# SonyCSLParis/interactive-spectrogram-inpainting

Hardware: AMD Instinct MI355X
Metric: spectrograms/sec VQ-VAE fwd+quantize @B64 (higher is better)
Workload: dtype f32 (products split into two f16 pieces, three terms); 1 GPU; VQVAE.forward (encode + quantize x2 + decode), eval, default ctor (128 hidden, 2 res blocks, D=64, K=512, factors 4/2); batch_per_gpu=64, input=[2,128,512] fp32 randn, weights=random init, codebooks calibrated on encoder outputs, parallelism=replicas x1 (no data-path collective)

## Files before the change

interactive-spectrogram-inpainting_amd/csrc/conv_first_f32.hip:

```cpp
#include <cstdlib>

#include "device_prims.h"
#include "isi_common.h"
#include "isi_internal.h"
#include "knobs.h"
#include "prof.h"
#include "split_f16.h"

namespace isi {

namespace {

constexpr unsigned OOB = 0xFFFFFFF0u;
constexpr int TILES_PER_WAVE = 8;
constexpr int LDT = 68;

struct FirstArgs {
  const float *in, *w, *bias;
  float *out;
  unsigned in_bytes;
  int s0n, s0c, s0h, s0w;
  int H, W, OH, OW, M;
  int relu, out_pair;
  float *out2;
  const float *gate;
  int32_t *zero;
  int zero_words;
};


template <int COUT>
__device__ __forceinline__ void store_tile(const FirstArgs &p, const float *tb, const int m0, const int lane) {
  if (p.out_pair) {
    constexpr int GP = COUT / 8;
    typedef unsigned u32x2v __attribute__((ext_vector_type(2)));
#pragma unroll
    for (int it = 0; it < 32 * GP / 64; ++it) {
      const int idx = it * 64 + lane;
      const int px = idx / GP, g = idx - px * GP;
      uint4 hi, lo;
      f16s::pair8_encode(*reinterpret_cast<const float4 *>(tb + px * LDT + g * 8),
                         *reinterpret_cast<const float4 *>(tb + px * LDT + g * 8 + 4), hi, lo);
      if (!p.out2 && 32 * GP % 64 == 0) {
        const u32x2v sx = __builtin_amdgcn_permlane32_swap(hi.x, lo.x, false, false);
        const u32x2v sy = __builtin_amdgcn_permlane32_swap(hi.y, lo.y, false, false);
        const u32x2v sz = __builtin_amdgcn_permlane32_swap(hi.z, lo.z, false, false);
        const u32x2v sw = __builtin_amdgcn_permlane32_swap(hi.w, lo.w, false, false);
        const uint4 first = make_uint4(sx.x, sy.x, sz.x, sw.x), second = make_uint4(sx.y, sy.y, sz.y, sw.y);
        const int up = lane >> 5;
        const int idx_a = it * 64 + (lane & 31), idx_b = idx_a + 32;
        const int pa = idx_a / GP, ga = idx_a - pa * GP, pb = idx_b / GP, gb = idx_b - pb * GP;
        if (m0 + pa < p.M) reinterpret_cast<uint4 *>(p.out + (size_t)(m0 + pa) * COUT + ga * 8)[up] = first;
        if (m0 + pb < p.M) reinterpret_cast<uint4 *>(p.out + (size_t)(m0 + pb) * COUT + gb * 8)[up] = second;
        continue;
      }
      if (m0 + px < p.M) {
        uint4 *o = reinterpret_cast<uint4 *>(p.out + (size_t)(m0 + px) * COUT + g * 8);
        o[0] = hi;
        o[1] = lo;
        if (p.out2) {
          float4 *o2 = reinterpret_cast<float4 *>(p.out2 + (size_t)(m0 + px) * COUT + g * 8);
          o2[0] = *reinterpret_cast<const float4 *>(tb + px * LDT + g * 8);
          o2[1] = *reinterpret_cast<const float4 *>(tb + px * LDT + g * 8 + 4);
        }
      }
    }
    return;
  }
  constexpr int QP = COUT / 4;
#pragma unroll
  for (int it = 0; it < 32 * QP / 64; ++it) {
    const int idx = it * 64 + lane;
    const int px = idx / QP, q = idx - px * QP;
    if (m0 + px < p.M) {
      float4 v = *reinterpret_cast<const float4 *>(tb + px * LDT + q * 4);
      if (p.gate) {
        const float4 g = *reinterpret_cast<const float4 *>(p.gate + (size_t)(m0 + px) * COUT + q * 4);
        v.x = g.x > 0.f ? v.x : 0.f; v.y = g.y > 0.f ? v.y : 0.f; v.z = g.z > 0.f ? v.z : 0.f; v.w = g.w > 0.f ? v.w : 0.f;
      }
      *reinterpret_cast<float4 *>(p.out + (size_t)(m0 + px) * COUT + q * 4) = v;
    }
  }
}

template <int NT>
__global__ __launch_bounds__(256) void conv_first_kernel(const FirstArgs p) {
  constexpr int COUT = NT * 32;
  __shared__ __attribute__((aligned(16))) float tbuf[4][32 * LDT];
  const int tid = threadIdx.x, lane = tid & 63, wave = tid >> 6;
  const int col = lane & 31, half = lane >> 5;
  float *tb = tbuf[wave];
  if (p.zero && blockIdx.x == 0)
    for (int i = tid; i < p.zero_words; i += 256) p.zero[i] = 0;

  float4 bw[4][NT];
#pragma unroll
  for (int s = 0; s < 4; ++s)
#pragma unroll
    for (int j = 0; j < NT; ++j)
      bw[s][j] = *reinterpret_cast<const float4 *>(p.w + (size_t)(32 * j + col) * 32 + 8 * s + 4 * half);
  float bias[NT];
#pragma unroll
  for (int j = 0; j < NT; ++j) bias[j] = p.bias ? p.bias[32 * j + col] : 0.f;

  const __amdgpu_buffer_rsrc_t rsi = __builtin_amdgcn_make_buffer_rsrc(const_cast<float *>(p.in), 0, p.in_bytes, 0x00020000);
  const int ohw = p.OH * p.OW;

  for (int t = 0; t < TILES_PER_WAVE; ++t) {
    const int tile = (t * (int)gridDim.x + (int)blockIdx.x) * 4 + wave;
    const int m0 = tile * 32;
    const int m = m0 + col;
    float a[4][4];
    {
      const bool ok = m < p.M;
      const int b = ok ? m / ohw : 0;
      const int rem = m - b * ohw;
      const int oy = rem / p.OW, ox = rem - oy * p.OW;
      const int iy0 = 2 * oy - 1, ix0 = 2 * ox - 1 + 2 * half;
      const int base = b * p.s0n;
#pragma unroll
      for (int s = 0; s < 4; ++s) {
        const int iy = iy0 + s;
        const bool yok = ok && (unsigned)iy < (unsigned)p.H;
#pragma unroll
        for (int e = 0; e < 4; ++e) {
          const int ix = ix0 + (e >> 1);
          const bool in_range = yok && (unsigned)ix < (unsigned)p.W;
          const unsigned off = in_range ? (unsigned)(base + (e & 1) * p.s0c + iy * p.s0h + ix * p.s0w) * 4u : OOB;
          a[s][e] = __builtin_bit_cast(float, __builtin_amdgcn_raw_buffer_load_b32(rsi, off, 0, 0));
        }
      }
    }
    f32x16 acc[NT];
#pragma unroll
    for (int j = 0; j < NT; ++j)
#pragma unroll
      for (int r = 0; r < 16; ++r) acc[j][r] = 0.f;
#pragma unroll
    for (int s = 0; s < 4; ++s)
#pragma unroll
      for (int e = 0; e < 4; ++e)
#pragma unroll
        for (int j = 0; j < NT; ++j) {
          const float bv = e == 0 ? bw[s][j].x : e == 1 ? bw[s][j].y : e == 2 ? bw[s][j].z : bw[s][j].w;
          acc[j] = __builtin_amdgcn_mfma_f32_32x32x2f32(a[s][e], bv, acc[j], 0, 0, 0);
        }
    __syncthreads();
#pragma unroll
    for (int j = 0; j < NT; ++j)
#pragma unroll
      for (int r = 0; r < 16; ++r) {
        const int row = (r & 3) + 8 * (r >> 2) + 4 * half;
        float v = acc[j][r] + bias[j];
        if (p.relu) v = fmaxf(v, 0.f) + (v - v);
        tb[row * LDT + 32 * j + col] = v;
      }
    __syncthreads();
    store_tile<COUT>(p, tb, m0, lane);
  }
}

typedef short s16x8f __attribute__((ext_vector_type(8)));
template <int NT>
__global__ __launch_bounds__(256) void conv_first_f16x3_kernel(const FirstArgs p) {
  constexpr int COUT = NT * 32;
  __shared__ __attribute__((aligned(16))) float tbuf[4][32 * LDT];
  const int tid = threadIdx.x, lane = tid & 63, wave = tid >> 6;
  const int col = lane & 31, half = lane >> 5;
  float *tb = tbuf[wave];
  if (p.zero && blockIdx.x == 0)
    for (int i = tid; i < p.zero_words; i += 256) p.zero[i] = 0;

  s16x8f bh[2][NT], bl[2][NT];
#pragma unroll
  for (int st = 0; st < 2; ++st)
#pragma unroll
    for (int j = 0; j < NT; ++j) {
      const float *wr = p.w + (size_t)(32 * j + col) * 32 + 16 * st + 8 * half;
      uint2 h0, l0, h1, l1;
      f16s::split4(*reinterpret_cast<const float4 *>(wr), f16s::kScaleB, h0, l0);
      f16s::split4(*reinterpret_cast<const float4 *>(wr + 4), f16s::kScaleB, h1, l1);
      bh[st][j] = __builtin_bit_cast(s16x8f, make_uint4(h0.x, h0.y, h1.x, h1.y));
      bl[st][j] = __builtin_bit_cast(s16x8f, make_uint4(l0.x, l0.y, l1.x, l1.y));
    }
  float bias[NT];
#pragma unroll
  for (int j = 0; j < NT; ++j) bias[j] = p.bias ? p.bias[32 * j + col] : 0.f;

  const __amdgpu_buffer_rsrc_t rsi = __builtin_amdgcn_make_buffer_rsrc(const_cast<float *>(p.in), 0, p.in_bytes, 0x00020000);
  const int ohw = p.OH * p.OW;

  for (int t = 0; t < TILES_PER_WAVE; ++t) {
    const int tile = (t * (int)gridDim.x + (int)blockIdx.x) * 4 + wave;
    const int m0 = tile * 32;
    const int m = m0 + col;
    float a[2][8];
    {
      const bool ok = m < p.M;
      const int b = ok ? m / ohw : 0;
      const int rem = m - b * ohw;
      const int oy = rem / p.OW, ox = rem - oy * p.OW;
      const int iy0 = 2 * oy - 1 + half, ix0 = 2 * ox - 1;
      const int base = b * p.s0n;
#pragma unroll
      for (int st = 0; st < 2; ++st) {
        const int iy = iy0 + 2 * st;
        const bool yok = ok && (unsigned)iy < (unsigned)p.H;
#pragma unroll
        for (int i = 0; i < 8; ++i) {
          const int ix = ix0 + (i >> 1);
          const bool in_range = yok && (unsigned)ix < (unsigned)p.W;
          const unsigned off = in_range ? (unsigned)(base + (i & 1) * p.s0c + iy * p.s0h + ix * p.s0w) * 4u : OOB;
          a[st][i] = __builtin_bit_cast(float, __builtin_amdgcn_raw_buffer_load_b32(rsi, off, 0, 0));
        }
      }
    }
    f32x16 acc[NT];
#pragma unroll
    for (int j = 0; j < NT; ++j)
#pragma unroll
      for (int r = 0; r < 16; ++r) acc[j][r] = 0.f;
#pragma unroll
    for (int st = 0; st < 2; ++st) {
      uint2 h0, l0, h1, l1;
      f16s::split4(make_float4(a[st][0], a[st][1], a[st][2], a[st][3]), f16s::kScaleA, h0, l0);
      f16s::split4(make_float4(a[st][4], a[st][5], a[st][6], a[st][7]), f16s::kScaleA, h1, l1);
      const s16x8f ah = __builtin_bit_cast(s16x8f, make_uint4(h0.x, h0.y, h1.x, h1.y));
      const s16x8f al = __builtin_bit_cast(s16x8f, make_uint4(l0.x, l0.y, l1.x, l1.y));
#pragma unroll
      for (int j = 0; j < NT; ++j) {
        acc[j] = __builtin_amdgcn_mfma_f32_32x32x16_f16(__builtin_bit_cast(f16s::f16x8, al), __builtin_bit_cast(f16s::f16x8, bh[st][j]), acc[j], 0, 0, 0);
        acc[j] = __builtin_amdgcn_mfma_f32_32x32x16_f16(__builtin_bit_cast(f16s::f16x8, ah), __builtin_bit_cast(f16s::f16x8, bl[st][j]), acc[j], 0, 0, 0);
        acc[j] = __builtin_amdgcn_mfma_f32_32x32x16_f16(__builtin_bit_cast(f16s::f16x8, ah), __builtin_bit_cast(f16s::f16x8, bh[st][j]), acc[j], 0, 0, 0);
      }
    }
    __syncthreads();
#pragma unroll
    for (int j = 0; j < NT; ++j)
#pragma unroll
      for (int r = 0; r < 16; ++r) {
        const int row = (r & 3) + 8 * (r >> 2) + 4 * half;
        float v = acc[j][r] * f16s::kUnscale + bias[j];
        if (p.relu) v = fmaxf(v, 0.f) + (v - v);
        tb[row * LDT + 32 * j + col] = v;
      }
    __syncthreads();
    store_tile<COUT>(p, tb, m0, lane);
  }
}

template <int NT, bool F16>
int launch_first(const FirstArgs &a, hipStream_t stream) {
  const int tiles = (a.M + 31) / 32;
  const int per_wg = 4 * TILES_PER_WAVE;
  dim3 grid((tiles + per_wg - 1) / per_wg);
  const double flops = 2.0 * a.M * (NT * 32) * 32;
  const double bytes = 4.0 * ((double)a.M / (a.OH * a.OW) * 2.0 * a.H * a.W + (double)a.M * NT * 32 + NT * 32 * 32);
  prof::Scope scope(prof::K_CONV_GATHER, flops, bytes, stream);
  if (F16) {
    ISI_PROF_LAUNCH(scope, conv_first_f16x3_kernel<NT>, grid, dim3(256), 0, stream, a);
  } else {
    ISI_PROF_LAUNCH(scope, conv_first_kernel<NT>, grid, dim3(256), 0, stream, a);
  }
  return check_launch("conv_first_f32");
}

}

bool conv_first_applicable(const isi_src *s0, const isi_src *s1, const isi_src *res, const isi_dst *dst, int Cout,
                           int KH, int KW, int stride, int pad, int OH, int OW, int nz) {
  const bool off = knobs().no_conv_first != 0;
  if (off || nz != 1 || (s1 && s1->ptr) || (res && res->ptr)) return false;
  if (s0->C != 2 || KH != 4 || KW != 4 || stride != 2 || pad != 1) return false;
  if (Cout != 32 && Cout != 64) return false;
  if (dst->sc != 1 || dst->sw != Cout || dst->sh != (int64_t)OW * Cout || dst->sn != (int64_t)OH * OW * Cout) return false;
  return (reinterpret_cast<uintptr_t>(dst->ptr) & 15) == 0;
}

int conv_first_f32(const isi_src *s0, const float *packed_w, const float *bias, const isi_dst *dst, int B, int H,
                   int W, int Cout, int OH, int OW, int64_t in_extent, int flags, hipStream_t stream, float *twin,
                   const float *gate, int32_t *zero, int zero_words) {
  FirstArgs a;
  if (zero && zero_words <= 0) return invalid("conv_first: bad zeroing request");
  a.zero = zero; a.zero_words = zero ? zero_words : 0;
  if (twin && !(flags & ISI_CONV_OUT_PAIR)) return unsupported("conv_first: an fp32 twin accompanies a pair-format output");
  if (gate && (flags & (ISI_CONV_OUT_PAIR | ISI_CONV_GATE_PAIR))) return unsupported("conv_first: the gated epilogue writes and reads fp32");
  a.out2 = twin; a.gate = gate;
  a.in = s0->ptr; a.w = packed_w; a.bias = bias; a.out = dst->ptr;
  a.in_bytes = (unsigned)(in_extent * 4);
  a.s0n = (int)s0->sn; a.s0c = (int)s0->sc; a.s0h = (int)s0->sh; a.s0w = (int)s0->sw;
  a.H = H; a.W = W; a.OH = OH; a.OW = OW; a.M = B * OH * OW;
  a.relu = flags & ISI_CONV_RELU; a.out_pair = (flags & ISI_CONV_OUT_PAIR) ? 1 : 0;
  if ((flags & ISI_CONV_F16X3) && !(flags & ISI_CONV_BF16X6))
    return Cout == 64 ? launch_first<2, true>(a, stream) : launch_first<1, true>(a, stream);
  return Cout == 64 ? launch_first<2, false>(a, stream) : launch_first<1, false>(a, stream);
}

}
```

Measured before the change: 37650 spectrograms/s.

## Restructure first conv kernel: row-aligned tiles, vector loads with DPP halo, specialized epilogues

Reworks the first 4x4 stride-2 conv kernel. Tiles now map to 32-pixel row segments, walked incrementally without per-pixel divides. For contiguous inputs each lane does a 64-bit load plus one edge load, and neighbours are exchanged with DPP shifts instead of 16 scalar gathers. The epilogue is specialized by template on mode and ReLU. It swaps the MFMA operands so accumulators can be written transposed to LDS with only wave-local fences instead of block barriers. It also uses buffer stores, stages bias in LDS and prefetches the next tile's input in the f16x3 path. These changes cut address arithmetic, load count and synchronization, at the cost of many more kernel instantiations and more complex edge handling.

```diff
diff --git a/interactive-spectrogram-inpainting_amd/csrc/conv_first_f32.hip b/interactive-spectrogram-inpainting_amd/csrc/conv_first_f32.hip
--- a/interactive-spectrogram-inpainting_amd/csrc/conv_first_f32.hip
+++ b/interactive-spectrogram-inpainting_amd/csrc/conv_first_f32.hip
@@ -21,6 +21,8 @@
   unsigned in_bytes;
   int s0n, s0c, s0h, s0w;
   int H, W, OH, OW, M;
+  int tpr, tiles;
+  int contig;
   int relu, out_pair;
   float *out2;
   const float *gate;
@@ -28,70 +30,164 @@
   int zero_words;
 };
 
-
-template <int COUT>
-__device__ __forceinline__ void store_tile(const FirstArgs &p, const float *tb, const int m0, const int lane) {
-  if (p.out_pair) {
+struct TileWalk {
+  int b, oy, tx;
+  int db, doy, dtx;
+  __device__ __forceinline__ TileWalk(const FirstArgs &p, const int first, const int step) {
+    const int row = first / p.tpr;
+    tx = first - row * p.tpr; b = row / p.OH; oy = row - b * p.OH;
+    const int srow = step / p.tpr;
+    dtx = step - srow * p.tpr; db = srow / p.OH; doy = srow - db * p.OH;
+  }
+  __device__ __forceinline__ void advance(const FirstArgs &p) {
+    tx += dtx; oy += doy; b += db;
+    if (tx >= p.tpr) { tx -= p.tpr; ++oy; }
+    if (oy >= p.OH) { oy -= p.OH; ++b; }
+  }
+};
+
+__device__ __forceinline__ float wave_shr1(const float v) {
+  return __builtin_bit_cast(float, __builtin_amdgcn_update_dpp(0, __builtin_bit_cast(int, v), 0x138, 0xf, 0xf, false));
+}
+__device__ __forceinline__ float wave_shl1(const float v) {
+  return __builtin_bit_cast(float, __builtin_amdgcn_update_dpp(0, __builtin_bit_cast(int, v), 0x130, 0xf, 0xf, false));
+}
+
+struct EdgeLane {
+  bool ok; int ex;
+  __device__ __forceinline__ EdgeLane(const FirstArgs &p, const int col, const int ox0) {
+    ex = col == 0 ? 2 * ox0 - 1 : 2 * ox0 + 64;
+    ok = ((col == 0) | (col == 31)) & ((unsigned)ex < (unsigned)p.W);
+  }
+};
+__device__ __forceinline__ void row4_issue(const __amdgpu_buffer_rsrc_t rsi, const int rowoff, const bool yok, const bool pok,
+                                           const int col, const int ox0, const EdgeLane &el, float (&raw)[3]) {
+  typedef float f32x2v __attribute__((ext_vector_type(2)));
+  const unsigned moff = (yok & pok) ? (unsigned)(rowoff + 2 * (ox0 + col)) * 4u : OOB;
+  const unsigned eoff = (yok & el.ok) ? (unsigned)(rowoff + el.ex) * 4u : OOB;
+  const f32x2v v = __builtin_bit_cast(f32x2v, __builtin_amdgcn_raw_buffer_load_b64(rsi, moff, 0, 0));
+  raw[0] = v.x; raw[1] = v.y;
+  raw[2] = __builtin_bit_cast(float, __builtin_amdgcn_raw_buffer_load_b32(rsi, eoff, 0, 0));
+}
+__device__ __forceinline__ void row4_finish(const float (&raw)[3], const int col, float (&r)[4]) {
+  const float left = wave_shr1(raw[1]), right = wave_shl1(raw[0]);
+  r[0] = col == 0 ? raw[2] : left;
+  r[1] = raw[0];
+  r[2] = raw[1];
+  r[3] = col == 31 ? raw[2] : right;
+}
+template <int N>
+__device__ __forceinline__ void row_elems(const __amdgpu_buffer_rsrc_t rsi, const FirstArgs &p, const int rowoff, const bool yok,
+                                          const bool pok, const int ix0, float (&r)[N]) {
+#pragma unroll
+  for (int k = 0; k < N; ++k) {
+    const int ix = ix0 + k;
+    const bool in_range = yok & pok & ((unsigned)ix < (unsigned)p.W);
+    r[k] = __builtin_bit_cast(float, __builtin_amdgcn_raw_buffer_load_b32(rsi, in_range ? (unsigned)(rowoff + ix * p.s0w) * 4u : OOB, 0, 0));
+  }
+}
+
+enum { EPI_F32 = 0, EPI_GATE = 1, EPI_PAIR = 2, EPI_TWIN = 3 };
+__device__ __forceinline__ void wave_lds_fence() {
+  __builtin_amdgcn_fence(__ATOMIC_RELEASE, "wavefront", "local");
+  __builtin_amdgcn_wave_barrier();
+  __builtin_amdgcn_fence(__ATOMIC_ACQUIRE, "wavefront", "local");
+}
+template <int NT, int MODE, bool RELU, bool SCALED, class MM>
+__device__ __forceinline__ void epilogue(const MM &mm, const float *bsh, float *tb, const __amdgpu_buffer_rsrc_t rso,
+                                         const __amdgpu_buffer_rsrc_t rsx, const int lane) {
+  constexpr int COUT = NT * 32;
+  const int col = lane & 31, half = lane >> 5;
+  typedef unsigned u32x2v __attribute__((ext_vector_type(2)));
+#pragma unroll
+  for (int j = 0; j < NT; ++j) {
+    if (j) __builtin_amdgcn_sched_barrier(0);
+    const f32x16 acc = mm(j);
+#pragma unroll
+    for (int q = 0; q < 4; ++q) {
+      const float4 bq = *reinterpret_cast<const float4 *>(bsh + 32 * j + 8 * q + 4 * half);
+      float v[4];
+#pragma unroll
+      for (int e = 0; e < 4; ++e) {
+        float t = SCALED ? acc[4 * q + e] * f16s::kUnscale + elem(bq, e) : acc[4 * q + e] + elem(bq, e);
+        if (RELU) t = fmaxf(t, 0.f) + (t - t);
+        v[e] = t;
+      }
+      *reinterpret_cast<float4 *>(tb + col * LDT + 32 * j + 8 * q + 4 * half) = make_float4(v[0], v[1], v[2], v[3]);
+    }
+  }
+  wave_lds_fence();
+  if constexpr (MODE == EPI_PAIR || MODE == EPI_TWIN) {
     constexpr int GP = COUT / 8;
-    typedef unsigned u32x2v __attribute__((ext_vector_type(2)));
 #pragma unroll
     for (int it = 0; it < 32 * GP / 64; ++it) {
       const int idx = it * 64 + lane;
       const int px = idx / GP, g = idx - px * GP;
+      const float4 a = *reinterpret_cast<const float4 *>(tb + px * LDT + g * 8), b = *reinterpret_cast<const float4 *>(tb + px * LDT + g * 8 + 4);
       uint4 hi, lo;
-      f16s::pair8_encode(*reinterpret_cast<const float4 *>(tb + px * LDT + g * 8),
-                         *reinterpret_cast<const float4 *>(tb + px * LDT + g * 8 + 4), hi, lo);
-      if (!p.out2 && 32 * GP % 64 == 0) {
+      f16s::pair8_encode(a, b, hi, lo);
+      if constexpr (MODE == EPI_PAIR) {
         const u32x2v sx = __builtin_amdgcn_permlane32_swap(hi.x, lo.x, false, false);
         const u32x2v sy = __builtin_amdgcn_permlane32_swap(hi.y, lo.y, false, false);
         const u32x2v sz = __builtin_amdgcn_permlane32_swap(hi.z, lo.z, false, false);
         const u32x2v sw = __builtin_amdgcn_permlane32_swap(hi.w, lo.w, false, false);
-        const uint4 first = make_uint4(sx.x, sy.x, sz.x, sw.x), second = make_uint4(sx.y, sy.y, sz.y, sw.y);
-        const int up = lane >> 5;
-        const int idx_a = it * 64 + (lane & 31), idx_b = idx_a + 32;
-        const int pa = idx_a / GP, ga = idx_a - pa * GP, pb = idx_b / GP, gb = idx_b - pb * GP;
-        if (m0 + pa < p.M) reinterpret_cast<uint4 *>(p.out + (size_t)(m0 + pa) * COUT + ga * 8)[up] = first;
-        if (m0 + pb < p.M) reinterpret_cast<uint4 *>(p.out + (size_t)(m0 + pb) * COUT + gb * 8)[up] = second;
-        continue;
-      }
-      if (m0 + px < p.M) {
-        uint4 *o = reinterpret_cast<uint4 *>(p.out + (size_t)(m0 + px) * COUT + g * 8);
-        o[0] = hi;
-        o[1] = lo;
-        if (p.out2) {
-          float4 *o2 = reinterpret_cast<float4 *>(p.out2 + (size_t)(m0 + px) * COUT + g * 8);
-          o2[0] = *reinterpret_cast<const float4 *>(tb + px * LDT + g * 8);
-          o2[1] = *reinterpret_cast<const float4 *>(tb + px * LDT + g * 8 + 4);
-        }
-      }
-    }
-    return;
-  }
-  constexpr int QP = COUT / 4;
-#pragma unroll
-  for (int it = 0; it < 32 * QP / 64; ++it) {
-    const int idx = it * 64 + lane;
-    const int px = idx / QP, q = idx - px * QP;
-    if (m0 + px < p.M) {
+        const i32x4 first = {(int)sx.x, (int)sy.x, (int)sz.x, (int)sw.x}, second = {(int)sx.y, (int)sy.y, (int)sz.y, (int)sw.y};
+        const int idx_a = it * 64 + col, idx_b = idx_a + 32;
+        __builtin_amdgcn_raw_buffer_store_b128(first, rso, (unsigned)idx_a * 32u + (unsigned)half * 16u, 0, 0);
+        __builtin_amdgcn_raw_buffer_store_b128(second, rso, (unsigned)idx_b * 32u + (unsigned)half * 16u, 0, 0);
+      } else {
+        __builtin_amdgcn_raw_buffer_store_b128(__builtin_bit_cast(i32x4, hi), rso, (unsigned)idx * 32u, 0, 0);
+        __builtin_amdgcn_raw_buffer_store_b128(__builtin_bit_cast(i32x4, lo), rso, (unsigned)idx * 32u + 16u, 0, 0);
+        __builtin_amdgcn_raw_buffer_store_b128(__builtin_bit_cast(i32x4, a), rsx, (unsigned)idx * 32u, 0, 0);
+        __builtin_amdgcn_raw_buffer_store_b128(__builtin_bit_cast(i32x4, b), rsx, (unsigned)idx * 32u + 16u, 0, 0);
+      }
+    }
+  } else {
+    constexpr int QP = COUT / 4;
+#pragma unroll
+    for (int it = 0; it < 32 * QP / 64; ++it) {
+      const int idx = it * 64 + lane;
+      const int px = idx / QP, q = idx - px * QP;
       float4 v = *reinterpret_cast<const float4 *>(tb + px * LDT + q * 4);
-      if (p.gate) {
-        const float4 g = *reinterpret_cast<const float4 *>(p.gate + (size_t)(m0 + px) * COUT + q * 4);
+      if constexpr (MODE == EPI_GATE) {
+        const float4 g = buf_load4(rsx, (unsigned)idx * 16u);
         v.x = g.x > 0.f ? v.x : 0.f; v.y = g.y > 0.f ? v.y : 0.f; v.z = g.z > 0.f ? v.z : 0.f; v.w = g.w > 0.f ? v.w : 0.f;
       }
-      *reinterpret_cast<float4 *>(p.out + (size_t)(m0 + px) * COUT + q * 4) = v;
-    }
-  }
-}
-
-template <int NT>
-__global__ __launch_bounds__(256) void conv_first_kernel(const FirstArgs p) {
+      __builtin_amdgcn_raw_buffer_store_b128(__builtin_bit_cast(i32x4, v), rso, (unsigned)idx * 16u, 0, 0);
+    }
+  }
+  wave_lds_fence();
+}
+
+template <int NT, bool SCALED, int MODE, bool RELU, class MM>
+__device__ __forceinline__ void store_tile(const FirstArgs &p, const MM &mm, const float *bsh, float *tb, const int b,
+                                           const int oy, const int tx, const int lane) {
   constexpr int COUT = NT * 32;
+  const int ox0 = tx * 32;
+  const int npx = min(32, p.OW - ox0);
+  const size_t first = ((size_t)(b * p.OH + oy) * p.OW + ox0) * COUT;
+  const unsigned bytes = (unsigned)npx * COUT * 4u;
+  const float *x = MODE == EPI_TWIN ? p.out2 : MODE == EPI_GATE ? p.gate : nullptr;
+  const __amdgpu_buffer_rsrc_t rso = __builtin_amdgcn_make_buffer_rsrc(p.out + first, 0, bytes, 0x00020000);
+  const __amdgpu_buffer_rsrc_t rsx = __builtin_amdgcn_make_buffer_rsrc(const_cast<float *>(x ? x + first : p.out), 0, x ? bytes : 0u, 0x00020000);
+  epilogue<NT, MODE, RELU, SCALED>(mm, bsh, tb, rso, rsx, lane);
+}
+
+template <int COUT>
+__device__ __forceinline__ void stage_bias(const FirstArgs &p, float *bsh, const int tid) {
+  if (tid < COUT) bsh[tid] = p.bias ? p.bias[tid] : 0.f;
+}
+
+template <int NT, bool CONTIG, int MODE, bool RELU>
+__global__ __launch_bounds__(256, 4) void conv_first_kernel(const FirstArgs p) {
+  __shared__ __attribute__((aligned(16))) float bsh[NT * 32];
   __shared__ __attribute__((aligned(16))) float tbuf[4][32 * LDT];
-  const int tid = threadIdx.x, lane = tid & 63, wave = tid >> 6;
+  const int tid = threadIdx.x, lane = tid & 63;
+  const int wave = __builtin_amdgcn_readfirstlane(tid >> 6);
   const int col = lane & 31, half = lane >> 5;
-  float *tb = tbuf[wave];
   if (p.zero && blockIdx.x == 0)
     for (int i = tid; i < p.zero_words; i += 256) p.zero[i] = 0;
+  stage_bias<NT * 32>(p, bsh, tid);
 
   float4 bw[4][NT];
 #pragma unroll
@@ -99,78 +195,118 @@
 #pragma unroll
     for (int j = 0; j < NT; ++j)
       bw[s][j] = *reinterpret_cast<const float4 *>(p.w + (size_t)(32 * j + col) * 32 + 8 * s + 4 * half);
-  float bias[NT];
-#pragma unroll
-  for (int j = 0; j < NT; ++j) bias[j] = p.bias ? p.bias[32 * j + col] : 0.f;
+  float *tb = tbuf[wave];
+  __syncthreads();
 
   const __amdgpu_buffer_rsrc_t rsi = __builtin_amdgcn_make_buffer_rsrc(const_cast<float *>(p.in), 0, p.in_bytes, 0x00020000);
-  const int ohw = p.OH * p.OW;
-
-  for (int t = 0; t < TILES_PER_WAVE; ++t) {
-    const int tile = (t * (int)gridDim.x + (int)blockIdx.x) * 4 + wave;
-    const int m0 = tile * 32;
-    const int m = m0 + col;
+  const int step = (int)gridDim.x * 4;
+  int tile = (int)blockIdx.x * 4 + wave;
+  TileWalk pos(p, tile, step);
+  for (int t = 0; t < TILES_PER_WAVE && tile < p.tiles; ++t, tile += step, pos.advance(p)) {
+    const int ox0 = pos.tx * 32;
+    const bool pok = ox0 + col < p.OW;
     float a[4][4];
-    {
-      const bool ok = m < p.M;
-      const int b = ok ? m / ohw : 0;
-      const int rem = m - b * ohw;
-      const int oy = rem / p.OW, ox = rem - oy * p.OW;
-      const int iy0 = 2 * oy - 1, ix0 = 2 * ox - 1 + 2 * half;
-      const int base = b * p.s0n;
+    if constexpr (CONTIG) {
+      const EdgeLane el(p, col, ox0);
+      float raw[4][2][3];
 #pragma unroll
       for (int s = 0; s < 4; ++s) {
-        const int iy = iy0 + s;
-        const bool yok = ok && (unsigned)iy < (unsigned)p.H;
-#pragma unroll
-        for (int e = 0; e < 4; ++e) {
-          const int ix = ix0 + (e >> 1);
-          const bool in_range = yok && (unsigned)ix < (unsigned)p.W;
-          const unsigned off = in_range ? (unsigned)(base + (e & 1) * p.s0c + iy * p.s0h + ix * p.s0w) * 4u : OOB;
-          a[s][e] = __builtin_bit_cast(float, __builtin_amdgcn_raw_buffer_load_b32(rsi, off, 0, 0));
+        const int iy = 2 * pos.oy - 1 + s;
+#pragma unroll
+        for (int c = 0; c < 2; ++c)
+          row4_issue(rsi, pos.b * p.s0n + c * p.s0c + iy * p.s0h, (unsigned)iy < (unsigned)p.H, pok, col, ox0, el, raw[s][c]);
+      }
+#pragma unroll
+      for (int s = 0; s < 4; ++s)
+#pragma unroll
+        for (int c = 0; c < 2; ++c) {
+          float r[4];
+          row4_finish(raw[s][c], col, r);
+          a[s][c] = half ? r[2] : r[0];
+          a[s][2 + c] = half ? r[3] : r[1];
         }
-      }
-    }
-    f32x16 acc[NT];
-#pragma unroll
-    for (int j = 0; j < NT; ++j)
-#pragma unroll
-      for (int r = 0; r < 16; ++r) acc[j][r] = 0.f;
-#pragma unroll
-    for (int s = 0; s < 4; ++s)
-#pragma unroll
-      for (int e = 0; e < 4; ++e)
-#pragma unroll
-        for (int j = 0; j < NT; ++j) {
-          const float bv = e == 0 ? bw[s][j].x : e == 1 ? bw[s][j].y : e == 2 ? bw[s][j].z : bw[s][j].w;
-          acc[j] = __builtin_amdgcn_mfma_f32_32x32x2f32(a[s][e], bv, acc[j], 0, 0, 0);
+    } else {
+#pragma unroll
+      for (int s = 0; s < 4; ++s) {
+        const int iy = 2 * pos.oy - 1 + s;
+#pragma unroll
+        for (int c = 0; c < 2; ++c) {
+          float r[2];
+          row_elems<2>(rsi, p, pos.b * p.s0n + c * p.s0c + iy * p.s0h, (unsigned)iy < (unsigned)p.H, pok, 2 * (ox0 + col) - 1 + 2 * half, r);
+          a[s][c] = r[0];
+          a[s][2 + c] = r[1];
         }
-    __syncthreads();
-#pragma unroll
-    for (int j = 0; j < NT; ++j)
-#pragma unroll
-      for (int r = 0; r < 16; ++r) {
-        const int row = (r & 3) + 8 * (r >> 2) + 4 * half;
-        float v = acc[j][r] + bias[j];
-        if (p.relu) v = fmaxf(v, 0.f) + (v - v);
-        tb[row * LDT + 32 * j + col] = v;
-      }
-    __syncthreads();
-    store_tile<COUT>(p, tb, m0, lane);
+      }
+    }
+    const auto mm = [&](const int j) {
+      f32x16 acc;
+#pragma unroll
+      for (int r = 0; r < 16; ++r) acc[r] = 0.f;
+#pragma unroll
+      for (int s = 0; s < 4; ++s)
+#pragma unroll
+        for (int e = 0; e < 4; ++e)
+          acc = __builtin_amdgcn_mfma_f32_32x32x2f32(elem(bw[s][j], e), a[s][e], acc, 0, 0, 0);
+      return acc;
+    };
+    store_tile<NT, false, MODE, RELU>(p, mm, bsh, tb, pos.b, pos.oy, pos.tx, lane);
   }
 }
 
 typedef short s16x8f __attribute__((ext_vector_type(8)));
-template <int NT>
-__global__ __launch_bounds__(256) void conv_first_f16x3_kernel(const FirstArgs p) {
-  constexpr int COUT = NT * 32;
+
+template <bool CONTIG>
+__device__ __forceinline__ void tile_issue(const __amdgpu_buffer_rsrc_t rsi, const FirstArgs &p, const TileWalk &pos,
+                                           const int col, const int half, float (&raw)[4][4]) {
+  const int ox0 = pos.tx * 32;
+  const bool pok = ox0 + col < p.OW;
+  const EdgeLane el(p, col, ox0);
+#pragma unroll
+  for (int st = 0; st < 2; ++st) {
+    const int iy = 2 * pos.oy - 1 + half + 2 * st;
+    const bool yok = (unsigned)iy < (unsigned)p.H;
+#pragma unroll
+    for (int c = 0; c < 2; ++c) {
+      const int rowoff = pos.b * p.s0n + c * p.s0c + iy * p.s0h;
+      if constexpr (CONTIG) {
+        float r3[3];
+        row4_issue(rsi, rowoff, yok, pok, col, ox0, el, r3);
+        raw[2 * st + c][0] = r3[0]; raw[2 * st + c][1] = r3[1]; raw[2 * st + c][2] = r3[2];
+      } else {
+        row_elems<4>(rsi, p, rowoff, yok, pok, 2 * (ox0 + col) - 1, raw[2 * st + c]);
+      }
+    }
+  }
+}
+template <bool CONTIG>
+__device__ __forceinline__ void tile_finish(const FirstArgs &p, const float (&raw)[4][4], const int col, float (&a)[2][8]) {
+#pragma unroll
+  for (int st = 0; st < 2; ++st)
+#pragma unroll
+    for (int c = 0; c < 2; ++c) {
+      float r[4];
+      if constexpr (CONTIG) {
+        const float r3[3] = {raw[2 * st + c][0], raw[2 * st + c][1], raw[2 * st + c][2]};
+        row4_finish(r3, col, r);
+      } else {
+#pragma unroll
+        for (int i = 0; i < 4; ++i) r[i] = raw[2 * st + c][i];
+      }
+#pragma unroll
+      for (int kw = 0; kw < 4; ++kw) a[st][2 * kw + c] = r[kw];
+    }
+}
+
+template <int NT, bool CONTIG, int MODE, bool RELU>
+__global__ __launch_bounds__(256, 4) void conv_first_f16x3_kernel(const FirstArgs p) {
+  __shared__ __attribute__((aligned(16))) float bsh[NT * 32];
   __shared__ __attribute__((aligned(16))) float tbuf[4][32 * LDT];
-  const int tid = threadIdx.x, lane = tid & 63, wave = tid >> 6;
+  const int tid = threadIdx.x, lane = tid & 63;
+  const int wave = __builtin_amdgcn_readfirstlane(tid >> 6);
   const int col = lane & 31, half = lane >> 5;
-  float *tb = tbuf[wave];
   if (p.zero && blockIdx.x == 0)
     for (int i = tid; i < p.zero_words; i += 256) p.zero[i] = 0;
-
+  stage_bias<NT * 32>(p, bsh, tid);
   s16x8f bh[2][NT], bl[2][NT];
 #pragma unroll
   for (int st = 0; st < 2; ++st)
@@ -183,86 +319,84 @@
       bh[st][j] = __builtin_bit_cast(s16x8f, make_uint4(h0.x, h0.y, h1.x, h1.y));
       bl[st][j] = __builtin_bit_cast(s16x8f, make_uint4(l0.x, l0.y, l1.x, l1.y));
     }
-  float bias[NT];
-#pragma unroll
-  for (int j = 0; j < NT; ++j) bias[j] = p.bias ? p.bias[32 * j + col] : 0.f;
+  float *tb = tbuf[wave];
+  __syncthreads();
 
   const __amdgpu_buffer_rsrc_t rsi = __builtin_amdgcn_make_buffer_rsrc(const_cast<float *>(p.in), 0, p.in_bytes, 0x00020000);
-  const int ohw = p.OH * p.OW;
-
-  for (int t = 0; t < TILES_PER_WAVE; ++t) {
-    const int tile = (t * (int)gridDim.x + (int)blockIdx.x) * 4 + wave;
-    const int m0 = tile * 32;
-    const int m = m0 + col;
+  const int step = (int)gridDim.x * 4;
+  int tile = (int)blockIdx.x * 4 + wave;
+  TileWalk pos(p, tile, step);
+  float raw[4][4];
+  if (tile < p.tiles) tile_issue<CONTIG>(rsi, p, pos, col, half, raw);
+  for (int t = 0; t < TILES_PER_WAVE && tile < p.tiles; ++t) {
     float a[2][8];
-    {
-      const bool ok = m < p.M;
-      const int b = ok ? m / ohw : 0;
-      const int rem = m - b * ohw;
-      const int oy = rem / p.OW, ox = rem - oy * p.OW;
-      const int iy0 = 2 * oy - 1 + half, ix0 = 2 * ox - 1;
-      const int base = b * p.s0n;
-#pragma unroll
-      for (int st = 0; st < 2; ++st) {
-        const int iy = iy0 + 2 * st;
-        const bool yok = ok && (unsigned)iy < (unsigned)p.H;
-#pragma unroll
-        for (int i = 0; i < 8; ++i) {
-          const int ix = ix0 + (i >> 1);
-          const bool in_range = yok && (unsigned)ix < (unsigned)p.W;
-          const unsigned off = in_range ? (unsigned)(base + (i & 1) * p.s0c + iy * p.s0h + ix * p.s0w) * 4u : OOB;
-          a[st][i] = __builtin_bit_cast(float, __builtin_amdgcn_raw_buffer_load_b32(rsi, off, 0, 0));
-        }
-      }
-    }
-    f32x16 acc[NT];
-#pragma unroll
-    for (int j = 0; j < NT; ++j)
-#pragma unroll
-      for (int r = 0; r < 16; ++r) acc[j][r] = 0.f;
+    tile_finish<CONTIG>(p, raw, col, a);
+    s16x8f ah[2], al[2];
 #pragma unroll
     for (int st = 0; st < 2; ++st) {
       uint2 h0, l0, h1, l1;
       f16s::split4(make_float4(a[st][0], a[st][1], a[st][2], a[st][3]), f16s::kScaleA, h0, l0);
       f16s::split4(make_float4(a[st][4], a[st][5], a[st][6], a[st][7]), f16s::kScaleA, h1, l1);
-      const s16x8f ah = __builtin_bit_cast(s16x8f, make_uint4(h0.x, h0.y, h1.x, h1.y));
-      const s16x8f al = __builtin_bit_cast(s16x8f, make_uint4(l0.x, l0.y, l1.x, l1.y));
-#pragma unroll
-      for (int j = 0; j < NT; ++j) {
-        acc[j] = __builtin_amdgcn_mfma_f32_32x32x16_f16(__builtin_bit_cast(f16s::f16x8, al), __builtin_bit_cast(f16s::f16x8, bh[st][j]), acc[j], 0, 0, 0);
-        acc[j] = __builtin_amdgcn_mfma_f32_32x32x16_f16(__builtin_bit_cast(f16s::f16x8, ah), __builtin_bit_cast(f16s::f16x8, bl[st][j]), acc[j], 0, 0, 0);
-        acc[j] = __builtin_amdgcn_mfma_f32_32x32x16_f16(__builtin_bit_cast(f16s::f16x8, ah), __builtin_bit_cast(f16s::f16x8, bh[st][j]), acc[j], 0, 0, 0);
-      }
-    }
-    __syncthreads();
-#pragma unroll
-    for (int j = 0; j < NT; ++j)
-#pragma unroll
-      for (int r = 0; r < 16; ++r) {
-        const int row = (r & 3) + 8 * (r >> 2) + 4 * half;
-        float v = acc[j][r] * f16s::kUnscale + bias[j];
-        if (p.relu) v = fmaxf(v, 0.f) + (v - v);
-        tb[row * LDT + 32 * j + col] = v;
-      }
-    __syncthreads();
-    store_tile<COUT>(p, tb, m0, lane);
-  }
-}
-
-template <int NT, bool F16>
-int launch_first(const FirstArgs &a, hipStream_t stream) {
-  const int tiles = (a.M + 31) / 32;
+      ah[st] = __builtin_bit_cast(s16x8f, make_uint4(h0.x, h0.y, h1.x, h1.y));
+      al[st] = __builtin_bit_cast(s16x8f, make_uint4(l0.x, l0.y, l1.x, l1.y));
+    }
+    const int b = pos.b, oy = pos.oy, tx = pos.tx;
+    tile += step;
+    pos.advance(p);
+    if (t + 1 < TILES_PER_WAVE && tile < p.tiles) tile_issue<CONTIG>(rsi, p, pos, col, half, raw);
+    const auto mm = [&](const int j) {
+      f32x16 acc;
+#pragma unroll
+      for (int r = 0; r < 16; ++r) acc[r] = 0.f;
+#pragma unroll
+      for (int st = 0; st < 2; ++st) {
+        acc = __builtin_amdgcn_mfma_f32_32x32x16_f16(__builtin_bit_cast(f16s::f16x8, bh[st][j]), __builtin_bit_cast(f16s::f16x8, al[st]), acc, 0, 0, 0);
+        acc = __builtin_amdgcn_mfma_f32_32x32x16_f16(__builtin_bit_cast(f16s::f16x8, bl[st][j]), __builtin_bit_cast(f16s::f16x8, ah[st]), acc, 0, 0, 0);
+        acc = __builtin_amdgcn_mfma_f32_32x32x16_f16(__builtin_bit_cast(f16s::f16x8, bh[st][j]), __builtin_bit_cast(f16s::f16x8, ah[st]), acc, 0, 0, 0);
+      }
+      return acc;
+    };
+    store_tile<NT, true, MODE, RELU>(p, mm, bsh, tb, b, oy, tx, lane);
+#pragma unroll
+    for (int i = 0; i < 4; ++i)
+#pragma unroll
+      for (int k = 0; k < 4; ++k) asm volatile("" : "+v"(raw[i][k]));
+  }
+}
+
+template <int NT, bool F16, bool CONTIG, int MODE, bool RELU>
+int launch_one(const FirstArgs &a, hipStream_t stream) {
   const int per_wg = 4 * TILES_PER_WAVE;
-  dim3 grid((tiles + per_wg - 1) / per_wg);
+  dim3 grid((a.tiles + per_wg - 1) / per_wg);
   const double flops = 2.0 * a.M * (NT * 32) * 32;
   const double bytes = 4.0 * ((double)a.M / (a.OH * a.OW) * 2.0 * a.H * a.W + (double)a.M * NT * 32 + NT * 32 * 32);
   prof::Scope scope(prof::K_CONV_GATHER, flops, bytes, stream);
   if (F16) {
-    ISI_PROF_LAUNCH(scope, conv_first_f16x3_kernel<NT>, grid, dim3(256), 0, stream, a);
+    ISI_PROF_LAUNCH(scope, (conv_first_f16x3_kernel<NT, CONTIG, MODE, RELU>), grid, dim3(256), 0, stream, a);
   } else {
-    ISI_PROF_LAUNCH(scope, conv_first_kernel<NT>, grid, dim3(256), 0, stream, a);
+    ISI_PROF_LAUNCH(scope, (conv_first_kernel<NT, CONTIG, MODE, RELU>), grid, dim3(256), 0, stream, a);
   }
   return check_launch("conv_first_f32");
+}
+
+template <int NT, bool F16, bool CONTIG>
+int launch_epilogue(const FirstArgs &a, hipStream_t stream) {
+  const int mode = a.out_pair ? (a.out2 ? EPI_TWIN : EPI_PAIR) : (a.gate ? EPI_GATE : EPI_F32);
+  switch (mode * 2 + (a.relu ? 1 : 0)) {
+    case EPI_F32 * 2:      return launch_one<NT, F16, CONTIG, EPI_F32, false>(a, stream);
+    case EPI_F32 * 2 + 1:  return launch_one<NT, F16, CONTIG, EPI_F32, true>(a, stream);
+    case EPI_GATE * 2:     return launch_one<NT, F16, CONTIG, EPI_GATE, false>(a, stream);
+    case EPI_GATE * 2 + 1: return launch_one<NT, F16, CONTIG, EPI_GATE, true>(a, stream);
+    case EPI_PAIR * 2:     return launch_one<NT, F16, CONTIG, EPI_PAIR, false>(a, stream);
+    case EPI_PAIR * 2 + 1: return launch_one<NT, F16, CONTIG, EPI_PAIR, true>(a, stream);
+    case EPI_TWIN * 2:     return launch_one<NT, F16, CONTIG, EPI_TWIN, false>(a, stream);
+    default:               return launch_one<NT, F16, CONTIG, EPI_TWIN, true>(a, stream);
+  }
+}
+
+template <int NT, bool F16>
+int launch_first(const FirstArgs &a, hipStream_t stream) {
+  return a.contig ? launch_epilogue<NT, F16, true>(a, stream) : launch_epilogue<NT, F16, false>(a, stream);
 }
 
 }
@@ -290,6 +424,8 @@
   a.in_bytes = (unsigned)(in_extent * 4);
   a.s0n = (int)s0->sn; a.s0c = (int)s0->sc; a.s0h = (int)s0->sh; a.s0w = (int)s0->sw;
   a.H = H; a.W = W; a.OH = OH; a.OW = OW; a.M = B * OH * OW;
+  a.tpr = (OW + 31) / 32; a.tiles = B * OH * a.tpr;
+  a.contig = a.s0w == 1 && W == 2 * OW && (reinterpret_cast<uintptr_t>(a.in) & 7) == 0 && !(a.s0n & 1) && !(a.s0c & 1) && !(a.s0h & 1);
   a.relu = flags & ISI_CONV_RELU; a.out_pair = (flags & ISI_CONV_OUT_PAIR) ? 1 : 0;
   if ((flags & ISI_CONV_F16X3) && !(flags & ISI_CONV_BF16X6))
     return Cout == 64 ? launch_first<2, true>(a, stream) : launch_first<1, true>(a, stream);
```

Measured after the change: 37990 spectrograms/s, median of 6. No clear change (+0.9%).
